# MrGiovanni/R-Super

Hardware: AMD Instinct MI355X
Metric: CT voxels/sec/node (96³ patch, bs=2/GPU) (higher is better)
Workload: dtype bf16; 1 GPU; R-Super 3D UNet(base 32, 26 classes, BasicBlock/IN) full training step (fwd + masked BCE + Dice loss + bwd + clip + AdamW + EMA), 96^3 patches, batch 2/GPU (BASELINE.json configs[1]); global_batch=2, patch=96, parallelism=dp1, sanity_checks_form=device-side flags read one step late (train_ddp.StepGuard)

## Files before the change

include/rsuper_hip.h:

```cpp
#ifndef RSUPER_HIP_H
#define RSUPER_HIP_H
#include <stddef.h>
#include <stdint.h>
#ifdef __cplusplus
extern "C" {
#endif

#define RSUPER_F32 0
#define RSUPER_BF16 1
#define RSUPER_OK 0
#define RSUPER_ERR_ARG 1
#define RSUPER_ERR_LAUNCH 2
#define RSUPER_ERR_UNSUPPORTED 3
#define RSUPER_ERR_NO_DEVICE 4

const char* rsuper_version(void);
int rsuper_device_check(void);


size_t rsuper_conv3_packed_elems(int dtype, int ka, int kb, int n_cols, int bn);

int rsuper_conv3_pack_weights(int dtype, int mode, const float* wa, const float* wb, int ka, int kb, int na, int nb,
                              int bn, void* packed, void* stream);

// ... 56 lines not shown

int rsuper_conv3_wgrad_s2_splits(int dtype, int Ca, int Mtot, int N, int FD, int FH, int FW);
int rsuper_conv3_wgrad_s2(int dtype, const void* xa, int lda, int Ca, const float* mra,
                          const void* ya, int ldya, int Ya, const void* yb, int ldyb, int Yb,
                          float* dwa, float* dwb, float* workspace, int N, int FD, int FH, int FW, int splits, void* stream);

size_t rsuper_pointwise_packed_bytes(int dtype, int K, int N);
int rsuper_pointwise(int dtype, int mode, const float* x, int ldx, const float* w, const float* bias, const float* res, int ldr,
                     float* y, int ldy, long R, int K, int N, void* packed, void* stream);
int rsuper_pointwise_pack_batch(int dtype, const long long* table, int n, long total_items, void* arena, void* stream);
int rsuper_pointwise_wgrad_splits(long R, int N, int K);
int rsuper_pointwise_wgrad(int dtype, const float* dy, int ldy, const float* x, int ldx, long R, int N, int K, float* workspace, int splits,
                           float* dw, float* db, void* stream);

int rsuper_stats_finalize(const float* part, int N, int nblk, int C, double cnt, float eps, int mode, int split, float* out, void* stream);
int rsuper_in_bwd_finalize(int dtype, const void* g, int ldg, const void* x, int ldx, const float* mr, const float* gm,
                           const void* add1, int lda1, const void* add2, int lda2, void* out, int ldo,
                           int N, int vox, int C, void* stream);

int rsuper_maxpool2_fwd(int dtype, const void* x, int ldx, void* y, int ldy, float* part, int blocks,
                        int N, int D, int H, int W, int C, void* stream);
int rsuper_maxpool2_bwd(int dtype, const void* x, int ldx, const void* dy, int lddy, void* dx, int lddx,
                        int N, int D, int H, int W, int C, void* stream);
int rsuper_maxpool2_bwd_add(int dtype, const void* x, int ldx, const void* dy, int lddy, const void* add, int lda, void* dx, int lddx,
                            int N, int D, int H, int W, int C, void* stream);

int rsuper_subsample2_fwd(int dtype, const void* x, int ldx, void* y, int ldy, float* part, int blocks,
                          int N, int D, int H, int W, int C, void* stream);
int rsuper_subsample2_bwd(int dtype, const void* dy, int lddy, void* dx, int lddx, int N, int D, int H, int W, int C, void* stream);

// ... 127 lines not shown
```

r-super_amd/csrc/api.hip:

```cpp
#include <string.h>
#include <math.h>
#include <stdlib.h>
#include "common.hpp"
#include "kernels.hpp"
#include "misc.hpp"
#include "loss.hpp"
#include "morph.hpp"
#include "optim.hpp"
#include "../../include/rsuper_hip.h"

#define ST(s) ((hipStream_t)(s))

static inline bool dt_ok(int dt) { return dt == RS_F32 || dt == RS_BF16; }
static inline bool ch_ok(int C, int ld) { return C >= 0 && (C % 8) == 0 && (ld % 8) == 0 && ld >= C; }
static inline bool bn_ok(int bn) { return bn == 32 || bn == 64 || bn == 96 || bn == 128; }
static inline int ntiles_for(int n_cols, int bn) { const int per = bn / 32; return ((n_cols + bn - 1) / bn) * per; }
static inline int pack_cols(int mode, int na, int nb) { return mode == 1 ? (nb ? (nb & 0xFFFF) : na) : na + nb; }
static inline bool pack_range_ok(int mode, int na, int nb) { return mode != 1 || nb == 0 || ((nb >> 16) % 32 == 0 && (nb & 0xFFFF) > 0 && (nb >> 16) + (nb & 0xFFFF) <= na); }

#include "igemm_plan.hpp"

template <typename F>
static int for_chunks(int n, void* const* p, void* const* g, void* const* m, void* const* v, void* const* e, const size_t* numel, F f) {
    for (int i0 = 0; i0 < n; i0 += RS_MT_MAX) {
// ... 342 lines not shown
}
int rsuper_pointwise_wgrad_splits(long R, int N, int K) { return (R > 0 && R <= 0x7FFFFFFFl && N > 0 && K > 0) ? rs_pw_wgrad_splits((int)R, N, K) : 0; }
int rsuper_pointwise_wgrad(int dtype, const float* dy, int ldy, const float* x, int ldx, long R, int N, int K, float* workspace, int splits,
                           float* dw, float* db, void* stream) {
    if (!dt_ok(dtype) || !dy || !x || !workspace || !dw || R <= 0 || N <= 0 || K <= 0 || splits <= 0) return RS_ERR_ARG;
    if ((N % 4) || (K % 4) || ldy < N || ldx < K) return RS_ERR_ARG;
    if ((unsigned long long)(R + 1) * ldx * 4ull >= (1ull << 32) || (unsigned long long)(R + 1) * ldy * 4ull >= (1ull << 32)) return RS_ERR_UNSUPPORTED;
    return rs_launch_pointwise_wgrad(dtype, dy, ldy, x, ldx, (int)R, N, K, workspace, splits, dw, db, ST(stream));
}

int rsuper_stats_finalize(const float* part, int N, int nblk, int C, double cnt, float eps, int mode, int split, float* out, void* stream) {
    if (!part || !out || N <= 0 || nblk <= 0 || C <= 0 || cnt <= 0 || split < 0 || split >= C || (mode != 0 && mode != 1)) return RS_ERR_ARG;
    return rs_launch_stats_finalize(part, N, nblk, C, cnt, eps, mode, split, out, ST(stream));
}

int rsuper_in_bwd_finalize(int dtype, const void* g, int ldg, const void* x, int ldx, const float* mr, const float* gm,
                           const void* add1, int lda1, const void* add2, int lda2, void* out, int ldo,
                           int N, int vox, int C, void* stream) {
    if (!dt_ok(dtype) || !g || !x || !mr || !gm || !out || !ch_ok(C, ldg) || !ch_ok(C, ldx) || !ch_ok(C, ldo)) return RS_ERR_ARG;
    InBwdParams p = {g, ldg, x, ldx, mr, gm, add1, lda1, add2, lda2, out, ldo, N, vox, C};
    return rs_launch_in_bwd(p, dtype, ST(stream));
}

int rsuper_maxpool2_fwd(int dtype, const void* x, int ldx, void* y, int ldy, float* part, int blocks,
                        int N, int D, int H, int W, int C, void* stream) {
    if (!dt_ok(dtype) || !x || !y || !ch_ok(C, ldx) || !ch_ok(C, ldy) || blocks <= 0 || D < 2 || H < 2 || W < 2) return RS_ERR_ARG;
    PoolParams p = {x, ldx, y, ldy, nullptr, 0, part, N, D, H, W, C};
    return rs_launch_pool(p, dtype, 0, blocks, ST(stream));
}
int rsuper_maxpool2_bwd(int dtype, const void* x, int ldx, const void* dy, int lddy, void* dx, int lddx,
// ... 394 lines not shown
```

r-super_amd/csrc/loss.hip:

```cpp
#include "common.hpp"
#include "misc.hpp"
#include "loss.hpp"

namespace {

__device__ __forceinline__ void sig_bce(float x, float t, float& sg, float& bce) {
    const float e = __expf(-fabsf(x));
    const float r = __frcp_rn(1.f + e);
    sg = x >= 0.f ? r : e * r;
    bce = fmaxf(x, 0.f) - x * t + __logf(1.f + e);
}
__device__ __forceinline__ float sigmoidf(float x) { float s, b; sig_bce(x, 0.f, s, b); return s; }

__global__ __launch_bounds__(256) void plane_partials_fwd_kernel(PlaneParams p) {
    const int plane = blockIdx.y;
    const size_t base = (size_t)plane * p.V;
    const float* x = p.x + (size_t)plane * p.xstride;
    const uint8_t* t = p.tpk ? p.tpk + ((size_t)(plane / p.tC) * p.tP + (size_t)((plane % p.tC) >> 3)) * p.V : (p.t ? p.t + base : nullptr);
    const uint32_t tm8 = p.tpk ? (0x80u >> ((plane % p.tC) & 7)) : 0xFFu;
    const bool kskip = p.kinv && p.kflags && !p.kflags[plane];
    const uint8_t* k = (p.k && !kskip) ? p.k + base : nullptr;
    const int kinv = k ? p.kinv : 0;
    const float* w1 = p.w1 ? p.w1 + base : nullptr;
    const uint8_t* w2 = p.w2 ? p.w2 + base : nullptr;
    float s[6] = {0.f, 0.f, 0.f, 0.f, 0.f, 0.f};
    const bool vec_ok = (p.V & 3) == 0 && (p.xstride & 3) == 0;
    size_t i0 = ((size_t)blockIdx.x * 256 + threadIdx.x) * 4;
    const bool wide_ok = vec_ok && (p.V & 15) == 0 && !w1 &&
                         ((((uintptr_t)p.x | (uintptr_t)p.t | (uintptr_t)p.tpk | (uintptr_t)p.k | (uintptr_t)p.w2) & 15) == 0);
    if (wide_ok) {
        auto term = [&](float xv, uint32_t tb, uint32_t kb, uint32_t w2b) {
            const float tt = (tb & tm8) ? 1.f : 0.f, kk = ((kb != 0u) != (kinv != 0)) ? 1.f : 0.f;
            float sg, b;
            sig_bce(xv, tt, sg, b);
            b *= kk;
            s[0] += b; s[1] += sg * kk; s[2] += sg * tt * kk; s[3] += tt * kk; s[5] += b * (w2b ? 0.f : 1.f);
        };
        for (size_t i = ((size_t)blockIdx.x * 256 + threadIdx.x) * 16; i < (size_t)p.V; i += (size_t)gridDim.x * 256 * 16) {
            float4 q[4];
#pragma unroll
            for (int u = 0; u < 4; ++u) q[u] = *(const float4*)(x + i + 4 * u);
            const uint4 tq = t ? *(const uint4*)(t + i) : make_uint4(0, 0, 0, 0);
            const uint4 kq = k ? *(const uint4*)(k + i) : make_uint4(0x01010101u, 0x01010101u, 0x01010101u, 0x01010101u);
            const uint4 wq = w2 ? *(const uint4*)(w2 + i) : make_uint4(0, 0, 0, 0);
            const uint32_t tw[4] = {tq.x, tq.y, tq.z, tq.w}, kw[4] = {kq.x, kq.y, kq.z, kq.w}, ww[4] = {wq.x, wq.y, wq.z, wq.w};
#pragma unroll
            for (int u = 0; u < 4; ++u) {
                const float xv[4] = {q[u].x, q[u].y, q[u].z, q[u].w};
#pragma unroll
                for (int j = 0; j < 4; ++j) term(xv[j], (tw[u] >> (8 * j)) & 0xFFu, (kw[u] >> (8 * j)) & 0xFFu, (ww[u] >> (8 * j)) & 0xFFu);
            }
        }
        i0 = (size_t)p.V;
    }
    for (size_t i = i0; i < (size_t)p.V; i += (size_t)gridDim.x * 256 * 4) {
        float xv[4]; uint8_t tv[4] = {0, 0, 0, 0}, kv[4] = {1, 1, 1, 1}, w2v[4] = {0, 0, 0, 0}; float w1v[4] = {0.f, 0.f, 0.f, 0.f};
        const bool full = vec_ok && i + 4 <= (size_t)p.V;
        if (full) {
            const float4 q = *(const float4*)(x + i);
            xv[0] = q.x; xv[1] = q.y; xv[2] = q.z; xv[3] = q.w;
            if (t) { const uchar4 u = *(const uchar4*)(t + i); tv[0] = u.x; tv[1] = u.y; tv[2] = u.z; tv[3] = u.w; }
            if (k) { const uchar4 u = *(const uchar4*)(k + i); kv[0] = u.x; kv[1] = u.y; kv[2] = u.z; kv[3] = u.w; }
            if (w2) { const uchar4 u = *(const uchar4*)(w2 + i); w2v[0] = u.x; w2v[1] = u.y; w2v[2] = u.z; w2v[3] = u.w; }
            if (w1) { const float4 u = *(const float4*)(w1 + i); w1v[0] = u.x; w1v[1] = u.y; w1v[2] = u.z; w1v[3] = u.w; }
        }
#pragma unroll
// ... 251 lines not shown
}

int rs_plane_partials_blocks(size_t V) {
    int blocks = (int)((V + 4095) / 4096);
    if (blocks > 64) blocks = 64;
    if (blocks < 1) blocks = 1;
    return blocks;
}
int rs_launch_plane_sums_reduce(const double* pblk, int rows, int nb, float* out, hipStream_t st) {
    hipLaunchKernelGGL(plane_sums_reduce_kernel, dim3((unsigned)((rows * 6 + 255) / 256)), dim3(256), 0, st, pblk, rows, nb, out);
    return rs_check_launch();
}
int rs_launch_plane_partials(const PlaneParams& p, int planes, int bwd, hipStream_t st) {
    const int blocks = rs_plane_partials_blocks(p.V);
    if (!bwd) {
        hipLaunchKernelGGL(plane_partials_fwd_kernel, dim3(blocks, planes), dim3(256), 0, st, p);
    } else {
        int b2 = (int)((p.V + 1023) / 1024);
        if (b2 > 256) b2 = 256;
        hipLaunchKernelGGL(plane_partials_bwd_kernel, dim3(b2, planes), dim3(256), 0, st, p);
    }
    return rs_check_launch();
}

int rs_launch_seg_from_sums(const SegSumsParams& p, hipStream_t st) {
    hipLaunchKernelGGL(seg_from_sums_kernel, dim3(1), dim3(256), 0, st, p);
    return rs_check_launch();
}

int rs_launch_report_from_sums(const ReportSumsParams& p, int R, hipStream_t st) {
    hipLaunchKernelGGL(report_from_sums_kernel, dim3(1), dim3(64), 0, st, p, R);
// ... 19 lines not shown
```

r-super_amd/csrc/misc.hpp:

```cpp
#pragma once
#include <hip/hip_runtime.h>
#include <stddef.h>
#include <stdint.h>

struct InBwdParams {
    const void* g; int ldg;
    const void* x; int ldx;
    const float* mr;
    const float* gm;
    const void* add1; int lda1;
    const void* add2; int lda2;
    void* out; int ldo;
    int N, vox, C;
};

struct PoolParams {
    const void* x; int ldx;
    void* y; int ldy;
    void* dx; int lddx;
    float* part;
    int N, D, H, W, C;
    const void* add; int lda;
};

// ... 31 lines not shown
int rs_battn_chunks(int L, int heads);
int rs_launch_battn(const float* fqv, const float* mqv, float* fout, float* mout, float* lse, const float* dfo, const float* dmo,
                    float* dfqv, float* dmqv, float* part, float* pms, int B, int L, int T, int heads, int dh, float scale, int bwd,
                    hipStream_t st);
int rs_launch_se_forward(const float* x, const float* w1, const float* b1, const float* w2, const float* b2, float* part, float* ms, float* tab,
                         float* hbuf, float* y, int N, long vox, int C, int r, hipStream_t st);
int rs_launch_se_backward(const float* x, const float* dy, const float* ident, const float* w1, const float* w2, const float* ms, const float* tab,
                          const float* hbuf, float* part, float* gm, float* dz1buf, float* tab2, float* dx, float* dw1, float* db1, float* dw2,
                          float* db2, int N, long vox, int C, int r, hipStream_t st);
int rs_launch_cl_planar(const float* src, float* dst, int N, long vox, int C, int K, int dir, hipStream_t st);
int rs_depthwise_rows(long vox);
int rs_launch_depthwise(const float* x, const float* w, float* y, int N, int D, int H, int W, int C, int flip, hipStream_t st);
int rs_launch_depthwise_wgrad(const float* x, const float* dy, float* part, float* dw, int N, int D, int H, int W, int C, hipStream_t st);
int rs_launch_stats_finalize(const float* part, int N, int nblk, int C, double cnt, float eps, int mode, int split, float* out, hipStream_t st);
int rs_elem_blocks(size_t items);
int rs_launch_in_bwd(const InBwdParams& p, int dtype, hipStream_t st);
int rs_launch_pool(const PoolParams& p, int dtype, int bwd, int blocks, hipStream_t st);
int rs_launch_subsample(const PoolParams& p, int dtype, int bwd, int blocks, hipStream_t st);
int rs_launch_upsample(const UpParams& p, int dtype, int bwd, int blocks, hipStream_t st);
int rs_launch_stem(const StemParams& p, int dtype, int wgrad, hipStream_t st);
int rs_launch_head(const HeadParams& p, int dtype, int which, hipStream_t st);
```

r-super_amd/csrc/unet_misc.hip:

```cpp
#include <string.h>
#include "common.hpp"
#include "kernels.hpp"
#include "misc.hpp"

namespace {

__global__ __launch_bounds__(1024) void stats_finalize_kernel(const float* part, int nblk, int C, double cnt, float eps, int mode, int split, float* out) {
    __shared__ double red[32][32][2];
    const int n = blockIdx.y;
    const int cl = threadIdx.x & 31, g = threadIdx.x >> 5;
    const int c = blockIdx.x * 32 + cl;
    double s0 = 0.0, s1 = 0.0;
    if (c < C) {
        const float* base = part + ((size_t)n * nblk * C + c) * 2;
        int b = g;
        for (; b + 96 < nblk; b += 128) {
            const float2 v0 = *(const float2*)(base + (size_t)b * C * 2), v1 = *(const float2*)(base + (size_t)(b + 32) * C * 2);
            const float2 v2 = *(const float2*)(base + (size_t)(b + 64) * C * 2), v3 = *(const float2*)(base + (size_t)(b + 96) * C * 2);
            s0 += ((double)v0.x + (double)v1.x) + ((double)v2.x + (double)v3.x);
            s1 += ((double)v0.y + (double)v1.y) + ((double)v2.y + (double)v3.y);
        }
        for (; b < nblk; b += 32) {
            const float2 v = *(const float2*)(base + (size_t)b * C * 2);
            s0 += (double)v.x; s1 += (double)v.y;
// ... 82 lines not shown
            float a[KP];
            unpack16<T>(a1q, a);
#pragma unroll
            for (int j = 0; j < KP; ++j) o[j] += a[j];
        }
        if (a2p) {
            float a[KP];
            unpack16<T>(a2q, a);
#pragma unroll
            for (int j = 0; j < KP; ++j) o[j] += a[j];
        }
        *(uint4*)(op + (size_t)v * p.ldo + c) = pack16<T>(o);
    }
}

template <typename T>
__global__ void maxpool_fwd_kernel(PoolParams p) {
    constexpr int KP = Elem<T>::KP;
    const int CV = p.C / KP, VL = 256 / CV;
    const int vl = threadIdx.x / CV, s = threadIdx.x % CV;
    const bool active = vl < VL;
    const int n = blockIdx.y;
    const int OD = p.D / 2, OH = p.H / 2, OW = p.W / 2;
    const int ovox = OD * OH * OW;
    const int per_blk = (ovox + gridDim.x - 1) / gridDim.x;
    const int v0 = blockIdx.x * per_blk, v1 = min(ovox, v0 + per_blk);
    float s1[KP], s2[KP];
#pragma unroll
    for (int j = 0; j < KP; ++j) { s1[j] = 0.f; s2[j] = 0.f; }
    if (active)
// ... 5 lines not shown
#pragma unroll
            for (int k = 0; k < 8; ++k) {
                const int d = od * 2 + (k >> 2), h = oh * 2 + ((k >> 1) & 1), w = ow * 2 + (k & 1);
                float x[KP];
                unpack16<T>(*(const uint4*)((const T*)p.x + ((((size_t)n * p.D + d) * p.H + h) * p.W + w) * (size_t)p.ldx + s * KP), x);
#pragma unroll
                for (int j = 0; j < KP; ++j) m[j] = fmaxf(m[j], x[j]);
            }
            *(uint4*)((T*)p.y + ((size_t)n * ovox + v) * p.ldy + s * KP) = pack16<T>(m);
#pragma unroll
            for (int j = 0; j < KP; ++j) { s1[j] += m[j]; s2[j] += m[j] * m[j]; }
        }
    if (p.part) block_channel_sums<KP>(s1, s2, p.C, CV, VL, vl, s, active, p.part + ((size_t)n * gridDim.x + blockIdx.x) * p.C * 2);
}

template <typename T>
__global__ void maxpool_bwd_kernel(PoolParams p) {
    constexpr int KP = Elem<T>::KP;
    const int CV = p.C / KP;
    const int n = blockIdx.y;
    const int OD = p.D / 2, OH = p.H / 2, OW = p.W / 2;
    const size_t total = (size_t)OD * OH * OW * CV;
    for (size_t i = (size_t)blockIdx.x * blockDim.x + threadIdx.x; i < total; i += (size_t)gridDim.x * blockDim.x) {
        const int s = (int)(i % CV); const int v = (int)(i / CV);
        const int ow = v % OW, oh = (v / OW) % OH, od = v / (OW * OH);
        float x[8][KP], m[KP], dy[KP];
#pragma unroll
        for (int j = 0; j < KP; ++j) m[j] = -INFINITY;
#pragma unroll
        for (int k = 0; k < 8; ++k) {
// ... 19 lines not shown
            if (p.add) {
                float a[KP];
                unpack16<T>(*(const uint4*)((const T*)p.add + ((((size_t)n * p.D + d) * p.H + h) * p.W + w) * (size_t)p.lda + s * KP), a);
#pragma unroll
                for (int j = 0; j < KP; ++j) o[j] += a[j];
            }
            *(uint4*)((T*)p.dx + ((((size_t)n * p.D + d) * p.H + h) * p.W + w) * (size_t)p.lddx + s * KP) = pack16<T>(o);
        }
    }
}

template <typename T>
__global__ void subsample_fwd_kernel(PoolParams p) {
    constexpr int KP = Elem<T>::KP;
    const int CV = p.C / KP, VL = 256 / CV;
    const int vl = threadIdx.x / CV, s = threadIdx.x % CV;
    const bool active = vl < VL;
    const int n = blockIdx.y;
    const int OD = (p.D + 1) / 2, OH = (p.H + 1) / 2, OW = (p.W + 1) / 2;
    const int ovox = OD * OH * OW;
    const int per_blk = (ovox + gridDim.x - 1) / gridDim.x;
    const int v0 = blockIdx.x * per_blk, v1 = min(ovox, v0 + per_blk);
    float s1[KP], s2[KP];
#pragma unroll
    for (int j = 0; j < KP; ++j) { s1[j] = 0.f; s2[j] = 0.f; }
    if (active)
        for (int v = v0 + vl; v < v1; v += VL) {
            const int ow = v % OW, oh = (v / OW) % OH, od = v / (OW * OH);
            const uint4 q = *(const uint4*)((const T*)p.x + ((((size_t)n * p.D + 2 * od) * p.H + 2 * oh) * p.W + 2 * ow) * (size_t)p.ldx + s * KP);
            *(uint4*)((T*)p.y + ((size_t)n * ovox + v) * p.ldy + s * KP) = q;
            float m[KP];
            unpack16<T>(q, m);
#pragma unroll
            for (int j = 0; j < KP; ++j) { s1[j] += m[j]; s2[j] += m[j] * m[j]; }
        }
    if (p.part) block_channel_sums<KP>(s1, s2, p.C, CV, VL, vl, s, active, p.part + ((size_t)n * gridDim.x + blockIdx.x) * p.C * 2);
}

template <typename T>
__global__ void subsample_bwd_kernel(PoolParams p) {
    constexpr int KP = Elem<T>::KP;
    const int CV = p.C / KP;
    const int n = blockIdx.y;
    const int OH = (p.H + 1) / 2, OW = (p.W + 1) / 2, OD = (p.D + 1) / 2;
    const size_t total = (size_t)p.D * p.H * p.W * CV;
    for (size_t i = (size_t)blockIdx.x * blockDim.x + threadIdx.x; i < total; i += (size_t)gridDim.x * blockDim.x) {
        const int s = (int)(i % CV); const size_t v = i / CV;
        const int w = (int)(v % p.W), h = (int)((v / p.W) % p.H), d = (int)(v / ((size_t)p.W * p.H));
        uint4 q = make_uint4(0, 0, 0, 0);
        if (!((d | h | w) & 1))
            q = *(const uint4*)((const T*)p.y + (((size_t)n * OD + d / 2) * OH + h / 2) * OW * (size_t)p.ldy + (size_t)(w / 2) * p.ldy + s * KP);
// ... 201 lines not shown
                    unpack16<T>(q[k], x);
#pragma unroll
                    for (int j = 0; j < KP; ++j) acc[j] = fmaf(wt[k], x[j], acc[j]);
                }
            }
#pragma unroll
            for (int j = 0; j < KP; ++j) acc[j] = Elem<T>::rnd(acc[j]);
            *(uint4*)(yout + (size_t)v * p.ldy) = pack16<T>(acc);
#pragma unroll
            for (int j = 0; j < KP; ++j) { s1[j] += acc[j]; s2[j] += acc[j] * acc[j]; }
            ow += VL;
            while (ow >= p.OW) { ow -= p.OW; if (++oh == p.OH) { oh = 0; ++od; } }
        }
    }
    if (p.part) block_channel_sums<KP>(s1, s2, p.C, CV, VL, vl, s, active, p.part + ((size_t)n * gridDim.x + blockIdx.x) * p.C * 2);
}

constexpr int UP_MAXW = 12;
struct UpEnt { int lo, n; float w[UP_MAXW]; };
template <typename T, int NW>
__device__ __forceinline__ void up_bwd_rows(const UpParams& p, const UpEnt* td, const UpEnt* th, const UpEnt* tw, int n, uint32_t i0, uint32_t total,
                                            uint32_t stride) {
    constexpr int KP = Elem<T>::KP;
    const uint32_t CV = (uint32_t)p.C / KP;
    const uint32_t ovox = (uint32_t)(p.OD * p.OH * p.OW);
    const __amdgpu_buffer_rsrc_t rs = __builtin_amdgcn_make_buffer_rsrc((void*)((const T*)p.y + (size_t)n * ovox * p.ldy), 0,
                                                                        ovox * (uint32_t)p.ldy * (uint32_t)sizeof(T), 0x00020000);
    for (uint32_t i = i0; i < total; i += stride) {
        const uint32_t v = i / CV, s = i - v * CV;
        const uint32_t iw = v % (uint32_t)p.IW, t2 = v / (uint32_t)p.IW, ih = t2 % (uint32_t)p.IH, id = t2 / (uint32_t)p.IH;
// ... 628 lines not shown
    if (smem > 64 * 1024) (void)hipFuncSetAttribute((const void*)k, hipFuncAttributeMaxDynamicSharedMemorySize, (int)smem);
}

}

int rs_launch_stats_finalize(const float* part, int N, int nblk, int C, double cnt, float eps, int mode, int split, float* out, hipStream_t st) {
    hipLaunchKernelGGL(stats_finalize_kernel, dim3((C + 31) / 32, N), dim3(1024), 0, st, part, nblk, C, cnt, eps, mode, split, out);
    return rs_check_launch();
}

int rs_elem_blocks(size_t items) {
    size_t b = (items + 255) / 256;
    return (int)(b < 1 ? 1 : (b > 4096 ? 4096 : b));
}

int rs_launch_in_bwd(const InBwdParams& p, int dtype, hipStream_t st) {
    const int KP = dtype == RS_F32 ? 4 : 8;
    if ((size_t)p.vox * (p.C / KP) >= 0xFFFFFFFFull) return RS_ERR_UNSUPPORTED;
    const int blocks = rs_elem_blocks((size_t)p.vox * (p.C / KP));
    if (dtype == RS_F32) hipLaunchKernelGGL(in_bwd_finalize_kernel<float>, dim3(blocks, p.N), dim3(256), 0, st, p);
    else hipLaunchKernelGGL(in_bwd_finalize_kernel<bf16_t>, dim3(blocks, p.N), dim3(256), 0, st, p);
    return rs_check_launch();
}

int rs_launch_pool(const PoolParams& p, int dtype, int bwd, int blocks, hipStream_t st) {
    const int KP = dtype == RS_F32 ? 4 : 8;
    const int CV = p.C / KP;
    if (CV > 256) return RS_ERR_UNSUPPORTED;
    if (!bwd) {
        const size_t smem = (size_t)(256 / CV) * p.C * 2 * sizeof(float);
        if (dtype == RS_F32) hipLaunchKernelGGL(maxpool_fwd_kernel<float>, dim3(blocks, p.N), dim3(256), smem, st, p);
        else hipLaunchKernelGGL(maxpool_fwd_kernel<bf16_t>, dim3(blocks, p.N), dim3(256), smem, st, p);
    } else {
        const int b = rs_elem_blocks((size_t)(p.D / 2) * (p.H / 2) * (p.W / 2) * CV);
        if (dtype == RS_F32) hipLaunchKernelGGL(maxpool_bwd_kernel<float>, dim3(b, p.N), dim3(256), 0, st, p);
        else hipLaunchKernelGGL(maxpool_bwd_kernel<bf16_t>, dim3(b, p.N), dim3(256), 0, st, p);
    }
    return rs_check_launch();
}

int rs_launch_subsample(const PoolParams& p, int dtype, int bwd, int blocks, hipStream_t st) {
    const int KP = dtype == RS_F32 ? 4 : 8;
    const int CV = p.C / KP;
    if (CV > 256) return RS_ERR_UNSUPPORTED;
    if (!bwd) {
        const size_t smem = (size_t)(256 / CV) * p.C * 2 * sizeof(float);
        if (dtype == RS_F32) hipLaunchKernelGGL(subsample_fwd_kernel<float>, dim3(blocks, p.N), dim3(256), smem, st, p);
        else hipLaunchKernelGGL(subsample_fwd_kernel<bf16_t>, dim3(blocks, p.N), dim3(256), smem, st, p);
    } else {
        const int b = rs_elem_blocks((size_t)p.D * p.H * p.W * CV);
        if (dtype == RS_F32) hipLaunchKernelGGL(subsample_bwd_kernel<float>, dim3(b, p.N), dim3(256), 0, st, p);
        else hipLaunchKernelGGL(subsample_bwd_kernel<bf16_t>, dim3(b, p.N), dim3(256), 0, st, p);
    }
    return rs_check_launch();
}

static int launch_upsample_bwd4(const void* g, int ldg, void* dx, int lddx, int N, int ID, int IH, int IW, int OD, int OH, int OW, int C, hipStream_t st) {
    static const bool off = getenv("RSUPER_UPSAMPLE_BWD4") && atoi(getenv("RSUPER_UPSAMPLE_BWD4")) == 0;
    if (off || (C % 8) || N > 65535) return RS_ERR_UNSUPPORTED;
    if ((size_t)OD * OH * OW * (size_t)ldg * 2 >= 0xFFFFFFFFull) return RS_ERR_UNSUPPORTED;
    struct Memo { int k[6]; int ok, nmax; };
    static thread_local Memo memo[8] = {};
    static thread_local int memo_next = 0;
// ... 14 lines not shown
    const int nbx = (IW * (C / 8) + 255) / 256;
    const unsigned blocks = (unsigned)(((ID + 1) / 2) * ((IH + 1) / 2) * nbx);
    if (nmax <= 4) hipLaunchKernelGGL((upsample_bwd4_kernel<4>), dim3(blocks, N), dim3(256), 0, st, p, nbx);
    else hipLaunchKernelGGL((upsample_bwd4_kernel<6>), dim3(blocks, N), dim3(256), 0, st, p, nbx);
    return rs_check_launch();
}

int rs_launch_upsample(const UpParams& p, int dtype, int bwd, int blocks, hipStream_t st) {
    const int KP = dtype == RS_F32 ? 4 : 8;
    const int CV = p.C / KP;
    if (CV > 256) return RS_ERR_UNSUPPORTED;
    if (!bwd) {
        static const bool v1 = getenv("RSUPER_UPSAMPLE_V1") != nullptr;
        const size_t smem = (size_t)(256 / CV) * p.C * 2 * sizeof(float);
        const bool small = (size_t)p.N * p.ID * p.IH * p.IW * p.ldx < 0x7FFFFFFFull;
        if (v1 || !small) {
            if (dtype == RS_F32) hipLaunchKernelGGL(upsample_fwd_kernel<float>, dim3(blocks, p.N), dim3(256), smem, st, p);
            else hipLaunchKernelGGL(upsample_fwd_kernel<bf16_t>, dim3(blocks, p.N), dim3(256), smem, st, p);
        } else {
            if (dtype == RS_F32) hipLaunchKernelGGL(upsample_fwd2_kernel<float>, dim3(blocks, p.N), dim3(256), smem, st, p);
            else hipLaunchKernelGGL(upsample_fwd2_kernel<bf16_t>, dim3(blocks, p.N), dim3(256), smem, st, p);
        }
    } else {
        static const bool v1 = getenv("RSUPER_UPSAMPLE_V1") != nullptr;
        auto ratio = [](int O, int I) { return I > 1 ? (double)(O - 1) / (double)(I - 1) : (double)O; };
        const double rmax = fmax(ratio(p.OD, p.ID), fmax(ratio(p.OH, p.IH), ratio(p.OW, p.IW)));
        if (!v1 && 2.0 * rmax + 2.0 > (double)UP_MAXW + 1e-9) return RS_ERR_UNSUPPORTED;
        const int b = rs_elem_blocks((size_t)p.ID * p.IH * p.IW * CV);
        const size_t tab = (size_t)(p.ID + p.IH + p.IW) * sizeof(UpEnt);
        const bool small = (size_t)p.OD * p.OH * p.OW * p.ldy * (dtype == RS_F32 ? 4 : 2) < 0xFFFFFFFFull && (size_t)p.ID * p.IH * p.IW * CV < 0xFFFFFFFFull && tab <= 48 * 1024;
        if (!v1 && dtype == RS_BF16) {
            const int rc = launch_upsample_bwd4(p.y, p.ldy, p.dx, p.lddx, p.N, p.ID, p.IH, p.IW, p.OD, p.OH, p.OW, p.C, st);
            if (rc != RS_ERR_UNSUPPORTED) return rc;
// ... 94 lines not shown
```

r-super_amd/hip/lib.py:

```python
import ctypes
import os
from ctypes import c_int, c_long, c_longlong, c_size_t, c_float, c_double, c_void_p, c_uint32, c_uint

_HERE = os.path.dirname(os.path.abspath(__file__))
SO_PATH = os.path.join(os.path.dirname(_HERE), 'csrc', 'librsuper_hip.so')

F32, BF16 = 0, 1
_LIB = None

P = c_void_p
_SIGS = {
    'rsuper_version': (ctypes.c_char_p, []),
    'rsuper_device_check': (c_int, []),
    'rsuper_conv3_packed_elems': (c_size_t, [c_int] * 5),
    'rsuper_conv3_pack_weights': (c_int, [c_int, c_int, P, P, c_int, c_int, c_int, c_int, c_int, P, P]),
    'rsuper_conv3_pack_weights_batch': (c_int, [c_int, c_int, P, P, P, P, P, P]),
    'rsuper_conv3_tiles': (c_int, [c_int] * 3),
    'rsuper_conv3_variant': (c_int, [c_int]),
    'rsuper_conv3_wgrad2_min_tiles': (c_int, [c_int]),
    'rsuper_conv3_plan': (c_int, [c_int] * 11 + [P]),
    'rsuper_conv3_box_bn': (c_int, [c_int] * 6),
    'rsuper_conv3_kd_bn': (c_int, [c_int] * 8),
    'rsuper_conv3_set_workspace': (c_int, [P, c_size_t]),
    'rsuper_conv3_workspace_bytes': (c_size_t, []),
# ... 8 lines not shown
    'rsuper_conv3_wgrad': (c_int, [c_int, c_int, P, c_int, c_int, P, P, c_int, c_int, P, P, c_int, c_int, P, c_int, c_int,
                                   P, P, P, c_int, c_int, c_int, c_int, c_int, P]),
    'rsuper_conv3_wgrad_partial': (c_int, [c_int, c_int, P, c_int, c_int, P, P, c_int, c_int, P, P, c_int, c_int, P, c_int, c_int,
                                           P, c_int, c_int, c_int, c_int, c_int, P]),
    'rsuper_conv3_wgrad_reduce': (c_int, [P, c_int, c_int, c_int, c_int, P, P, P]),
    'rsuper_conv3_wgrad_reduce_batch': (c_int, [c_int, P, P, P, P, P, P, P, P]),
    'rsuper_conv3_wgrad_reduce_batch_stats': (c_int, [c_int, P, P, P, P, P, P, P, c_int, P, P, P, P, P, P, P, P, c_float, P]),
    'rsuper_conv3_wgrad_s2_splits': (c_int, [c_int] * 7),
    'rsuper_conv3_wgrad_s2': (c_int, [c_int, P, c_int, c_int, P, P, c_int, c_int, P, c_int, c_int, P, P, P, c_int, c_int, c_int, c_int, c_int, P]),
    'rsuper_pointwise_packed_bytes': (c_size_t, [c_int, c_int, c_int]),
    'rsuper_pointwise': (c_int, [c_int, c_int, P, c_int, P, P, P, c_int, P, c_int, c_long, c_int, c_int, P, P]),
    'rsuper_pointwise_pack_batch': (c_int, [c_int, P, c_int, c_long, P, P]),
    'rsuper_pointwise_wgrad_splits': (c_int, [c_long, c_int, c_int]),
    'rsuper_pointwise_wgrad': (c_int, [c_int, P, c_int, P, c_int, c_long, c_int, c_int, P, c_int, P, P, P]),
    'rsuper_stats_finalize': (c_int, [P, c_int, c_int, c_int, c_double, c_float, c_int, c_int, P, P]),
    'rsuper_in_bwd_finalize': (c_int, [c_int, P, c_int, P, c_int, P, P, P, c_int, P, c_int, P, c_int, c_int, c_int, c_int, P]),
    'rsuper_maxpool2_fwd': (c_int, [c_int, P, c_int, P, c_int, P, c_int, c_int, c_int, c_int, c_int, c_int, P]),
    'rsuper_maxpool2_bwd': (c_int, [c_int, P, c_int, P, c_int, P, c_int, c_int, c_int, c_int, c_int, c_int, P]),
    'rsuper_maxpool2_bwd_add': (c_int, [c_int, P, c_int, P, c_int, P, c_int, P, c_int, c_int, c_int, c_int, c_int, c_int, P]),
    'rsuper_subsample2_fwd': (c_int, [c_int, P, c_int, P, c_int, P, c_int, c_int, c_int, c_int, c_int, c_int, P]),
    'rsuper_subsample2_bwd': (c_int, [c_int, P, c_int, P, c_int, c_int, c_int, c_int, c_int, c_int, P]),
    'rsuper_upsample_fwd': (c_int, [c_int, P, c_int, P, c_int, P, c_int] + [c_int] * 8 + [P]),
    'rsuper_upsample_bwd': (c_int, [c_int, P, c_int, P, c_int] + [c_int] * 8 + [P]),
    'rsuper_stem_fwd': (c_int, [c_int, P, P, P, c_int, P, c_int, c_int, c_int, c_int, c_int, P]),
    'rsuper_stem_wgrad': (c_int, [c_int, P, P, c_int, P, c_int, c_int, c_int, c_int, c_int, P]),
    'rsuper_head_fwd': (c_int, [c_int, P, c_int, P, P, P, c_int, c_int, c_int, c_int, P]),
    'rsuper_head_bwd_data': (c_int, [c_int, P, P, P, c_int, c_int, c_int, c_int, c_int, P]),
    'rsuper_head_bwd_weight': (c_int, [c_int, P, c_int, P, P, P, c_int, c_int, c_int, c_int, P]),
    'rsuper_head_bwd': (c_int, [c_int, P, c_int, P, P, P, c_int, P, P, c_int, c_int, c_int, c_int, P]),
    'rsuper_plane_partials_fwd': (c_int, [P, c_size_t, P, P, P, P, P, c_int, c_int, c_size_t, P]),
# ... 105 lines not shown
```

Measured before the change: 172.0 million voxels/s.

## Add tuned glue kernel variants for pooling, upsample, IN backward and loss partials

Adds a runtime-switchable set of alternative glue kernels, enabled by default and disabled by setting RSUPER_GLUE_KERNELS=0. The set includes a software-pipelined loss partials kernel and an unrolled IN-backward finalize with batched loads. It also adds a maxpool forward with multi-voxel load batching, an upsample forward using shared-memory coordinate tables, and a channel split over gridDim.z for small-grid stat kernels. Maxpool backward uses smaller blocks for small grids. The aim is more memory-level parallelism and better occupancy on small late-stage tensors, at the cost of more code paths and extra partial-stat layout complexity.

```diff
diff --git a/include/rsuper_hip.h b/include/rsuper_hip.h
--- a/include/rsuper_hip.h
+++ b/include/rsuper_hip.h
@@ -94,6 +94,7 @@
                            float* dw, float* db, void* stream);
 
 int rsuper_stats_finalize(const float* part, int N, int nblk, int C, double cnt, float eps, int mode, int split, float* out, void* stream);
+int rsuper_glue_variant(int v);
 int rsuper_in_bwd_finalize(int dtype, const void* g, int ldg, const void* x, int ldx, const float* mr, const float* gm,
                            const void* add1, int lda1, const void* add2, int lda2, void* out, int ldo,
                            int N, int vox, int C, void* stream);
diff --git a/r-super_amd/csrc/api.hip b/r-super_amd/csrc/api.hip
--- a/r-super_amd/csrc/api.hip
+++ b/r-super_amd/csrc/api.hip
@@ -380,6 +380,8 @@
     return rs_launch_stats_finalize(part, N, nblk, C, cnt, eps, mode, split, out, ST(stream));
 }
 
+int rsuper_glue_variant(int v) { return rs_glue_variant(v); }
+
 int rsuper_in_bwd_finalize(int dtype, const void* g, int ldg, const void* x, int ldx, const float* mr, const float* gm,
                            const void* add1, int lda1, const void* add2, int lda2, void* out, int ldo,
                            int N, int vox, int C, void* stream) {
diff --git a/r-super_amd/csrc/loss.hip b/r-super_amd/csrc/loss.hip
--- a/r-super_amd/csrc/loss.hip
+++ b/r-super_amd/csrc/loss.hip
@@ -12,6 +12,7 @@
 }
 __device__ __forceinline__ float sigmoidf(float x) { float s, b; sig_bce(x, 0.f, s, b); return s; }
 
+template <bool PIPE>
 __global__ __launch_bounds__(256) void plane_partials_fwd_kernel(PlaneParams p) {
     const int plane = blockIdx.y;
     const size_t base = (size_t)plane * p.V;
@@ -36,20 +37,39 @@
             b *= kk;
             s[0] += b; s[1] += sg * kk; s[2] += sg * tt * kk; s[3] += tt * kk; s[5] += b * (w2b ? 0.f : 1.f);
         };
-        for (size_t i = ((size_t)blockIdx.x * 256 + threadIdx.x) * 16; i < (size_t)p.V; i += (size_t)gridDim.x * 256 * 16) {
-            float4 q[4];
-#pragma unroll
-            for (int u = 0; u < 4; ++u) q[u] = *(const float4*)(x + i + 4 * u);
-            const uint4 tq = t ? *(const uint4*)(t + i) : make_uint4(0, 0, 0, 0);
-            const uint4 kq = k ? *(const uint4*)(k + i) : make_uint4(0x01010101u, 0x01010101u, 0x01010101u, 0x01010101u);
-            const uint4 wq = w2 ? *(const uint4*)(w2 + i) : make_uint4(0, 0, 0, 0);
-            const uint32_t tw[4] = {tq.x, tq.y, tq.z, tq.w}, kw[4] = {kq.x, kq.y, kq.z, kq.w}, ww[4] = {wq.x, wq.y, wq.z, wq.w};
+        struct Trip { float4 q[4]; uint4 tq, kq, wq; };
+        auto fetch = [&](size_t i) {
+            Trip r;
+#pragma unroll
+            for (int u = 0; u < 4; ++u) r.q[u] = *(const float4*)(x + i + 4 * u);
+            r.tq = t ? *(const uint4*)(t + i) : make_uint4(0, 0, 0, 0);
+            r.kq = k ? *(const uint4*)(k + i) : make_uint4(0x01010101u, 0x01010101u, 0x01010101u, 0x01010101u);
+            r.wq = w2 ? *(const uint4*)(w2 + i) : make_uint4(0, 0, 0, 0);
+            return r;
+        };
+        auto eval = [&](const Trip& r) {
+            const uint32_t tw[4] = {r.tq.x, r.tq.y, r.tq.z, r.tq.w}, kw[4] = {r.kq.x, r.kq.y, r.kq.z, r.kq.w}, ww[4] = {r.wq.x, r.wq.y, r.wq.z, r.wq.w};
 #pragma unroll
             for (int u = 0; u < 4; ++u) {
-                const float xv[4] = {q[u].x, q[u].y, q[u].z, q[u].w};
+                const float xv[4] = {r.q[u].x, r.q[u].y, r.q[u].z, r.q[u].w};
 #pragma unroll
                 for (int j = 0; j < 4; ++j) term(xv[j], (tw[u] >> (8 * j)) & 0xFFu, (kw[u] >> (8 * j)) & 0xFFu, (ww[u] >> (8 * j)) & 0xFFu);
             }
+        };
+        const size_t step = (size_t)gridDim.x * 256 * 16;
+        size_t i = ((size_t)blockIdx.x * 256 + threadIdx.x) * 16;
+        if (PIPE) {
+            if (i < (size_t)p.V) {
+                Trip cur = fetch(i);
+                for (i += step; i < (size_t)p.V; i += step) {
+                    const Trip nxt = fetch(i);
+                    eval(cur);
+                    cur = nxt;
+                }
+                eval(cur);
+            }
+        } else {
+            for (; i < (size_t)p.V; i += step) eval(fetch(i));
         }
         i0 = (size_t)p.V;
     }
@@ -331,7 +351,8 @@
 int rs_launch_plane_partials(const PlaneParams& p, int planes, int bwd, hipStream_t st) {
     const int blocks = rs_plane_partials_blocks(p.V);
     if (!bwd) {
-        hipLaunchKernelGGL(plane_partials_fwd_kernel, dim3(blocks, planes), dim3(256), 0, st, p);
+        if (rs_glue_variant(-1)) hipLaunchKernelGGL(plane_partials_fwd_kernel<true>, dim3(blocks, planes), dim3(256), 0, st, p);
+        else hipLaunchKernelGGL(plane_partials_fwd_kernel<false>, dim3(blocks, planes), dim3(256), 0, st, p);
     } else {
         int b2 = (int)((p.V + 1023) / 1024);
         if (b2 > 256) b2 = 256;
diff --git a/r-super_amd/csrc/misc.hpp b/r-super_amd/csrc/misc.hpp
--- a/r-super_amd/csrc/misc.hpp
+++ b/r-super_amd/csrc/misc.hpp
@@ -69,6 +69,7 @@
 int rs_launch_depthwise_wgrad(const float* x, const float* dy, float* part, float* dw, int N, int D, int H, int W, int C, hipStream_t st);
 int rs_launch_stats_finalize(const float* part, int N, int nblk, int C, double cnt, float eps, int mode, int split, float* out, hipStream_t st);
 int rs_elem_blocks(size_t items);
+int rs_glue_variant(int v);
 int rs_launch_in_bwd(const InBwdParams& p, int dtype, hipStream_t st);
 int rs_launch_pool(const PoolParams& p, int dtype, int bwd, int blocks, hipStream_t st);
 int rs_launch_subsample(const PoolParams& p, int dtype, int bwd, int blocks, hipStream_t st);
diff --git a/r-super_amd/csrc/unet_misc.hip b/r-super_amd/csrc/unet_misc.hip
--- a/r-super_amd/csrc/unet_misc.hip
+++ b/r-super_amd/csrc/unet_misc.hip
@@ -120,6 +120,66 @@
     }
 }
 
+template <typename T, int U>
+__global__ __launch_bounds__(256) void in_bwd_finalize2_kernel(InBwdParams p, int cv_shift) {
+    constexpr int KP = Elem<T>::KP;
+    const uint32_t CV = 1u << cv_shift;
+    const uint32_t total = (uint32_t)p.vox * CV;
+    const uint32_t n = blockIdx.y;
+    const uint32_t i0 = blockIdx.x * (256u * U) + threadIdx.x;
+    if (i0 >= total) return;
+    const T* gp = (const T*)p.g + (size_t)n * p.vox * p.ldg;
+    const T* xp = (const T*)p.x + (size_t)n * p.vox * p.ldx;
+    const T* a1p = p.add1 ? (const T*)p.add1 + (size_t)n * p.vox * p.lda1 : nullptr;
+    const T* a2p = p.add2 ? (const T*)p.add2 + (size_t)n * p.vox * p.lda2 : nullptr;
+    T* op = (T*)p.out + (size_t)n * p.vox * p.ldo;
+    const uint32_t c = (i0 & (CV - 1u)) * KP;
+    uint4 gq[U], xq[U], a1q[U], a2q[U];
+#pragma unroll
+    for (int u = 0; u < U; ++u) {
+        const uint32_t i = i0 + 256u * u;
+        const uint32_t v = (i < total ? i : i0) >> cv_shift;
+        gq[u] = *(const uint4*)(gp + (size_t)v * p.ldg + c);
+        xq[u] = *(const uint4*)(xp + (size_t)v * p.ldx + c);
+        a1q[u] = make_uint4(0, 0, 0, 0); a2q[u] = make_uint4(0, 0, 0, 0);
+        if (a1p) a1q[u] = *(const uint4*)(a1p + (size_t)v * p.lda1 + c);
+        if (a2p) a2q[u] = *(const uint4*)(a2p + (size_t)v * p.lda2 + c);
+    }
+    float mu[KP], rs[KP], m1[KP], m2[KP];
+#pragma unroll
+    for (int j = 0; j < KP; ++j) {
+        const size_t o = ((size_t)n * p.C + c + j) * 2;
+        mu[j] = p.mr[o]; rs[j] = p.mr[o + 1]; m1[j] = p.gm[o]; m2[j] = p.gm[o + 1];
+    }
+#pragma unroll
+    for (int u = 0; u < U; ++u) {
+        const uint32_t i = i0 + 256u * u;
+        if (i >= total) break;
+        const uint32_t v = i >> cv_shift;
+        float g[KP], x[KP], o[KP];
+        unpack16<T>(gq[u], g);
+        unpack16<T>(xq[u], x);
+#pragma unroll
+        for (int j = 0; j < KP; ++j) {
+            const float xn = (x[j] - mu[j]) * rs[j];
+            o[j] = rs[j] * (g[j] - m1[j] - xn * m2[j]);
+        }
+        if (a1p) {
+            float a[KP];
+            unpack16<T>(a1q[u], a);
+#pragma unroll
+            for (int j = 0; j < KP; ++j) o[j] += a[j];
+        }
+        if (a2p) {
+            float a[KP];
+            unpack16<T>(a2q[u], a);
+#pragma unroll
+            for (int j = 0; j < KP; ++j) o[j] += a[j];
+        }
+        *(uint4*)(op + (size_t)v * p.ldo + c) = pack16<T>(o);
+    }
+}
+
 template <typename T>
 __global__ void maxpool_fwd_kernel(PoolParams p) {
     constexpr int KP = Elem<T>::KP;
@@ -155,6 +215,58 @@
     if (p.part) block_channel_sums<KP>(s1, s2, p.C, CV, VL, vl, s, active, p.part + ((size_t)n * gridDim.x + blockIdx.x) * p.C * 2);
 }
 
+template <typename T, int U>
+__global__ __launch_bounds__(256) void maxpool_fwd2_kernel(PoolParams p) {
+    constexpr int KP = Elem<T>::KP;
+    const int CV = p.C / KP, VL = 256 / CV;
+    const int CVb = CV / gridDim.z;
+    const int vl = threadIdx.x / CVb, s = blockIdx.z * CVb + threadIdx.x % CVb;
+    const bool active = vl < VL;
+    const int n = blockIdx.y;
+    const int OD = p.D / 2, OH = p.H / 2, OW = p.W / 2;
+    const int ovox = OD * OH * OW;
+    const int per_blk = (ovox + gridDim.x - 1) / gridDim.x;
+    const int v0 = blockIdx.x * per_blk, v1 = min(ovox, v0 + per_blk);
+    float s1[KP], s2[KP];
+#pragma unroll
+    for (int j = 0; j < KP; ++j) { s1[j] = 0.f; s2[j] = 0.f; }
+    if (active)
+        for (int v = v0 + vl; v < v1; v += U * VL) {
+            uint4 q[U][8];
+#pragma unroll
+            for (int u = 0; u < U; ++u) {
+                const int vv = v + u * VL < v1 ? v + u * VL : v;
+                const int ow = vv % OW, oh = (vv / OW) % OH, od = vv / (OW * OH);
+#pragma unroll
+                for (int k = 0; k < 8; ++k) {
+                    const int d = od * 2 + (k >> 2), h = oh * 2 + ((k >> 1) & 1), w = ow * 2 + (k & 1);
+                    q[u][k] = *(const uint4*)((const T*)p.x + ((((size_t)n * p.D + d) * p.H + h) * p.W + w) * (size_t)p.ldx + s * KP);
+                }
+            }
+#pragma unroll
+            for (int u = 0; u < U; ++u) {
+                if (v + u * VL >= v1) break;
+                float m[KP];
+#pragma unroll
+                for (int j = 0; j < KP; ++j) m[j] = -INFINITY;
+#pragma unroll
+                for (int k = 0; k < 8; ++k) {
+                    float x[KP];
+                    unpack16<T>(q[u][k], x);
+#pragma unroll
+                    for (int j = 0; j < KP; ++j) m[j] = fmaxf(m[j], x[j]);
+                }
+                *(uint4*)((T*)p.y + ((size_t)n * ovox + v + u * VL) * p.ldy + s * KP) = pack16<T>(m);
+#pragma unroll
+                for (int j = 0; j < KP; ++j) { s1[j] += m[j]; s2[j] = fmaf(m[j], m[j], s2[j]); }
+            }
+        }
+    const int Cb = CVb * KP;
+    if (p.part)
+        block_channel_sums<KP>(s1, s2, Cb, CVb, VL, vl, threadIdx.x % CVb, active,
+                               p.part + (((size_t)n * gridDim.x + blockIdx.x) * p.C + (size_t)blockIdx.z * Cb) * 2);
+}
+
 template <typename T>
 __global__ void maxpool_bwd_kernel(PoolParams p) {
     constexpr int KP = Elem<T>::KP;
@@ -204,7 +316,8 @@
 __global__ void subsample_fwd_kernel(PoolParams p) {
     constexpr int KP = Elem<T>::KP;
     const int CV = p.C / KP, VL = 256 / CV;
-    const int vl = threadIdx.x / CV, s = threadIdx.x % CV;
+    const int CVb = CV / gridDim.z;
+    const int vl = threadIdx.x / CVb, s = blockIdx.z * CVb + threadIdx.x % CVb;
     const bool active = vl < VL;
     const int n = blockIdx.y;
     const int OD = (p.D + 1) / 2, OH = (p.H + 1) / 2, OW = (p.W + 1) / 2;
@@ -224,7 +337,10 @@
 #pragma unroll
             for (int j = 0; j < KP; ++j) { s1[j] += m[j]; s2[j] += m[j] * m[j]; }
         }
-    if (p.part) block_channel_sums<KP>(s1, s2, p.C, CV, VL, vl, s, active, p.part + ((size_t)n * gridDim.x + blockIdx.x) * p.C * 2);
+    const int Cb = CVb * KP;
+    if (p.part)
+        block_channel_sums<KP>(s1, s2, Cb, CVb, VL, vl, threadIdx.x % CVb, active,
+                               p.part + (((size_t)n * gridDim.x + blockIdx.x) * p.C + (size_t)blockIdx.z * Cb) * 2);
 }
 
 template <typename T>
@@ -456,6 +572,100 @@
         }
     }
     if (p.part) block_channel_sums<KP>(s1, s2, p.C, CV, VL, vl, s, active, p.part + ((size_t)n * gridDim.x + blockIdx.x) * p.C * 2);
+}
+
+struct UpTab { uint32_t o0, o1; float l0, l1; };
+template <typename T>
+__global__ __launch_bounds__(256) void upsample_fwd3_kernel(UpParams p) {
+    extern __shared__ __attribute__((aligned(16))) char smem[];
+    constexpr int KP = Elem<T>::KP;
+    const int CV = p.C / KP, VL = 256 / CV;
+    const int CVb = CV / gridDim.z;
+    const int Cb = CVb * KP;
+    const int vl = threadIdx.x / CVb, s = blockIdx.z * CVb + threadIdx.x % CVb;
+    const bool active = vl < VL;
+    const int n = blockIdx.y;
+    const int ovox = p.OD * p.OH * p.OW;
+    const int per_blk = (ovox + gridDim.x - 1) / gridDim.x;
+    const int v0 = blockIdx.x * per_blk, v1 = min(ovox, v0 + per_blk);
+    const float sd = p.OD > 1 ? (float)(p.ID - 1) / (float)(p.OD - 1) : 0.f;
+    const float sh = p.OH > 1 ? (float)(p.IH - 1) / (float)(p.OH - 1) : 0.f;
+    const float sw = p.OW > 1 ? (float)(p.IW - 1) / (float)(p.OW - 1) : 0.f;
+    UpTab* tab = (UpTab*)(smem + (size_t)VL * Cb * 2 * sizeof(float));
+    for (int t = threadIdx.x; t < p.OD + p.OH + p.OW; t += blockDim.x) {
+        const int axis = t < p.OD ? 0 : (t < p.OD + p.OH ? 1 : 2);
+        const int o = axis == 0 ? t : (axis == 1 ? t - p.OD : t - p.OD - p.OH);
+        const float sc = axis == 0 ? sd : (axis == 1 ? sh : sw);
+        const int I = axis == 0 ? p.ID : (axis == 1 ? p.IH : p.IW);
+        const uint32_t stride = (uint32_t)sizeof(T) * (uint32_t)p.ldx * (axis == 0 ? (uint32_t)(p.IH * p.IW) : (axis == 1 ? (uint32_t)p.IW : 1u));
+        int i0, i1; float l;
+        lin_coord(o, sc, I, i0, i1, l);
+        UpTab e;
+        e.o0 = (uint32_t)i0 * stride; e.o1 = (uint32_t)i1 * stride; e.l0 = 1.f - l; e.l1 = l;
+        tab[t] = e;
+    }
+    __syncthreads();
+    const UpTab* td = tab; const UpTab* th = tab + p.OD; const UpTab* tw = tab + p.OD + p.OH;
+    float s1[KP], s2[KP];
+#pragma unroll
+    for (int j = 0; j < KP; ++j) { s1[j] = 0.f; s2[j] = 0.f; }
+    const char* xin = (const char*)((const T*)p.x + (size_t)n * p.ID * p.IH * p.IW * p.ldx + s * KP);
+    if (active && v0 + vl < v1) {
+        int v = v0 + vl;
+        int ow = v % p.OW, oh = (v / p.OW) % p.OH, od = v / (p.OW * p.OH);
+        T* yp = (T*)p.y + ((size_t)n * ovox + v) * p.ldy + s * KP;
+        const size_t ystep = (size_t)VL * p.ldy;
+        for (; v < v1; v += VL, yp += ystep) {
+            const UpTab ed = td[od], eh = th[oh], ew = tw[ow];
+            const uint32_t rows[4] = {ed.o0 + eh.o0, ed.o0 + eh.o1, ed.o1 + eh.o0, ed.o1 + eh.o1};
+            const float wdh[4] = {ed.l0 * eh.l0, ed.l0 * eh.l1, ed.l1 * eh.l0, ed.l1 * eh.l1};
+            uint4 q[8];
+            float wt[8];
+#pragma unroll
+            for (int k = 0; k < 8; ++k) {
+                q[k] = *(const uint4*)(xin + (rows[k >> 1] + ((k & 1) ? ew.o1 : ew.o0)));
+                wt[k] = wdh[k >> 1] * ((k & 1) ? ew.l1 : ew.l0);
+            }
+            float acc[KP];
+            if (sizeof(T) == 2) {
+                f32x2_t a2[4];
+#pragma unroll
+                for (int j = 0; j < 4; ++j) a2[j] = f32x2_t{0.f, 0.f};
+#pragma unroll
+                for (int k = 0; k < 8; ++k) {
+                    const uint32_t wq[4] = {q[k].x, q[k].y, q[k].z, q[k].w};
+                    const f32x2_t w2 = {wt[k], wt[k]};
+#pragma unroll
+                    for (int j = 0; j < 4; ++j) {
+                        const f32x2_t x2 = {__uint_as_float(wq[j] << 16), __uint_as_float(wq[j] & 0xffff0000u)};
+                        a2[j] = __builtin_elementwise_fma(w2, x2, a2[j]);
+                    }
+                }
+#pragma unroll
+                for (int j = 0; j < 4; ++j) { acc[2 * j] = a2[j][0]; acc[2 * j + 1] = a2[j][1]; }
+            } else {
+#pragma unroll
+                for (int j = 0; j < KP; ++j) acc[j] = 0.f;
+#pragma unroll
+                for (int k = 0; k < 8; ++k) {
+                    float x[KP];
+                    unpack16<T>(q[k], x);
+#pragma unroll
+                    for (int j = 0; j < KP; ++j) acc[j] = fmaf(wt[k], x[j], acc[j]);
+                }
+            }
+#pragma unroll
+            for (int j = 0; j < KP; ++j) acc[j] = Elem<T>::rnd(acc[j]);
+            *(uint4*)yp = pack16<T>(acc);
+#pragma unroll
+            for (int j = 0; j < KP; ++j) { s1[j] += acc[j]; s2[j] = fmaf(acc[j], acc[j], s2[j]); }
+            ow += VL;
+            while (ow >= p.OW) { ow -= p.OW; if (++oh == p.OH) { oh = 0; ++od; } }
+        }
+    }
+    if (p.part)
+        block_channel_sums<KP>(s1, s2, Cb, CVb, VL, vl, threadIdx.x % CVb, active,
+                               p.part + (((size_t)n * gridDim.x + blockIdx.x) * p.C + (size_t)blockIdx.z * Cb) * 2);
 }
 
 constexpr int UP_MAXW = 12;
@@ -1114,10 +1324,39 @@
     return (int)(b < 1 ? 1 : (b > 4096 ? 4096 : b));
 }
 
+int rs_glue_variant(int v) {
+    static int g = !(getenv("RSUPER_GLUE_KERNELS") && atoi(getenv("RSUPER_GLUE_KERNELS")) == 0);
+    if (v == 0 || v == 1) g = v;
+    return g;
+}
+
+static int stat_csplit(int rows, int N, int CV) {
+    if (!rs_glue_variant(-1)) return 1;
+    const int VL = 256 / CV;
+    int z = 1;
+    while ((size_t)rows * N * z < 1024 && CV % (2 * z) == 0 && CV / (2 * z) >= 8 && (CV / (2 * z)) * VL >= 64) z *= 2;
+    return z;
+}
+
 int rs_launch_in_bwd(const InBwdParams& p, int dtype, hipStream_t st) {
     const int KP = dtype == RS_F32 ? 4 : 8;
     if ((size_t)p.vox * (p.C / KP) >= 0xFFFFFFFFull) return RS_ERR_UNSUPPORTED;
     const int blocks = rs_elem_blocks((size_t)p.vox * (p.C / KP));
+    const uint32_t CV = (uint32_t)(p.C / KP);
+    const size_t nb1 = ((size_t)p.vox * CV + 255) / 256;
+    if (rs_glue_variant(-1) && CV > 0 && (CV & (CV - 1)) == 0 && CV <= 256 && nb1 >= 256 && nb1 <= 8192) {
+        const int sh = __builtin_ctz(CV);
+        if (nb1 >= 1024) {
+            const dim3 grid((unsigned)((nb1 + 3) / 4), p.N);
+            if (dtype == RS_F32) hipLaunchKernelGGL((in_bwd_finalize2_kernel<float, 4>), grid, dim3(256), 0, st, p, sh);
+            else hipLaunchKernelGGL((in_bwd_finalize2_kernel<bf16_t, 4>), grid, dim3(256), 0, st, p, sh);
+        } else {
+            const dim3 grid((unsigned)((nb1 + 1) / 2), p.N);
+            if (dtype == RS_F32) hipLaunchKernelGGL((in_bwd_finalize2_kernel<float, 2>), grid, dim3(256), 0, st, p, sh);
+            else hipLaunchKernelGGL((in_bwd_finalize2_kernel<bf16_t, 2>), grid, dim3(256), 0, st, p, sh);
+        }
+        return rs_check_launch();
+    }
     if (dtype == RS_F32) hipLaunchKernelGGL(in_bwd_finalize_kernel<float>, dim3(blocks, p.N), dim3(256), 0, st, p);
     else hipLaunchKernelGGL(in_bwd_finalize_kernel<bf16_t>, dim3(blocks, p.N), dim3(256), 0, st, p);
     return rs_check_launch();
@@ -1129,12 +1368,21 @@
     if (CV > 256) return RS_ERR_UNSUPPORTED;
     if (!bwd) {
         const size_t smem = (size_t)(256 / CV) * p.C * 2 * sizeof(float);
-        if (dtype == RS_F32) hipLaunchKernelGGL(maxpool_fwd_kernel<float>, dim3(blocks, p.N), dim3(256), smem, st, p);
-        else hipLaunchKernelGGL(maxpool_fwd_kernel<bf16_t>, dim3(blocks, p.N), dim3(256), smem, st, p);
+        if (rs_glue_variant(-1) && (size_t)blocks * p.N < 1024) {
+            const int z = stat_csplit(blocks, p.N, CV);
+            const dim3 grid(blocks, p.N, z), blk(z == 1 ? 256 : (CV / z) * (256 / CV));
+            if (dtype == RS_F32) hipLaunchKernelGGL((maxpool_fwd2_kernel<float, 4>), grid, blk, smem / z, st, p);
+            else hipLaunchKernelGGL((maxpool_fwd2_kernel<bf16_t, 4>), grid, blk, smem / z, st, p);
+        } else {
+            if (dtype == RS_F32) hipLaunchKernelGGL(maxpool_fwd_kernel<float>, dim3(blocks, p.N), dim3(256), smem, st, p);
+            else hipLaunchKernelGGL(maxpool_fwd_kernel<bf16_t>, dim3(blocks, p.N), dim3(256), smem, st, p);
+        }
     } else {
-        const int b = rs_elem_blocks((size_t)(p.D / 2) * (p.H / 2) * (p.W / 2) * CV);
-        if (dtype == RS_F32) hipLaunchKernelGGL(maxpool_bwd_kernel<float>, dim3(b, p.N), dim3(256), 0, st, p);
-        else hipLaunchKernelGGL(maxpool_bwd_kernel<bf16_t>, dim3(b, p.N), dim3(256), 0, st, p);
+        const size_t items = (size_t)(p.D / 2) * (p.H / 2) * (p.W / 2) * CV;
+        int b = rs_elem_blocks(items), threads = 256;
+        if (rs_glue_variant(-1) && (size_t)b * p.N < 512) { threads = 64; b = (int)((items + 63) / 64); }
+        if (dtype == RS_F32) hipLaunchKernelGGL(maxpool_bwd_kernel<float>, dim3(b, p.N), dim3(threads), 0, st, p);
+        else hipLaunchKernelGGL(maxpool_bwd_kernel<bf16_t>, dim3(b, p.N), dim3(threads), 0, st, p);
     }
     return rs_check_launch();
 }
@@ -1145,8 +1393,10 @@
     if (CV > 256) return RS_ERR_UNSUPPORTED;
     if (!bwd) {
         const size_t smem = (size_t)(256 / CV) * p.C * 2 * sizeof(float);
-        if (dtype == RS_F32) hipLaunchKernelGGL(subsample_fwd_kernel<float>, dim3(blocks, p.N), dim3(256), smem, st, p);
-        else hipLaunchKernelGGL(subsample_fwd_kernel<bf16_t>, dim3(blocks, p.N), dim3(256), smem, st, p);
+        const int z = stat_csplit(blocks, p.N, CV);
+        const dim3 grid(blocks, p.N, z), blk(z == 1 ? 256 : (CV / z) * (256 / CV));
+        if (dtype == RS_F32) hipLaunchKernelGGL(subsample_fwd_kernel<float>, grid, blk, smem / z, st, p);
+        else hipLaunchKernelGGL(subsample_fwd_kernel<bf16_t>, grid, blk, smem / z, st, p);
     } else {
         const int b = rs_elem_blocks((size_t)p.D * p.H * p.W * CV);
         if (dtype == RS_F32) hipLaunchKernelGGL(subsample_bwd_kernel<float>, dim3(b, p.N), dim3(256), 0, st, p);
@@ -1191,9 +1441,16 @@
         static const bool v1 = getenv("RSUPER_UPSAMPLE_V1") != nullptr;
         const size_t smem = (size_t)(256 / CV) * p.C * 2 * sizeof(float);
         const bool small = (size_t)p.N * p.ID * p.IH * p.IW * p.ldx < 0x7FFFFFFFull;
+        const size_t tab3 = (size_t)(p.OD + p.OH + p.OW) * sizeof(UpTab);
+        const bool fwd3 = rs_glue_variant(-1) && small && (size_t)p.ID * p.IH * p.IW * p.ldx * (dtype == RS_F32 ? 4 : 2) < 0xFFFFFFFFull && smem + tab3 <= 64 * 1024;
         if (v1 || !small) {
             if (dtype == RS_F32) hipLaunchKernelGGL(upsample_fwd_kernel<float>, dim3(blocks, p.N), dim3(256), smem, st, p);
             else hipLaunchKernelGGL(upsample_fwd_kernel<bf16_t>, dim3(blocks, p.N), dim3(256), smem, st, p);
+        } else if (fwd3) {
+            const int z = stat_csplit(blocks, p.N, CV);
+            const dim3 grid(blocks, p.N, z), blk(z == 1 ? 256 : (CV / z) * (256 / CV));
+            if (dtype == RS_F32) hipLaunchKernelGGL(upsample_fwd3_kernel<float>, grid, blk, smem / z + tab3, st, p);
+            else hipLaunchKernelGGL(upsample_fwd3_kernel<bf16_t>, grid, blk, smem / z + tab3, st, p);
         } else {
             if (dtype == RS_F32) hipLaunchKernelGGL(upsample_fwd2_kernel<float>, dim3(blocks, p.N), dim3(256), smem, st, p);
             else hipLaunchKernelGGL(upsample_fwd2_kernel<bf16_t>, dim3(blocks, p.N), dim3(256), smem, st, p);
diff --git a/r-super_amd/hip/lib.py b/r-super_amd/hip/lib.py
--- a/r-super_amd/hip/lib.py
+++ b/r-super_amd/hip/lib.py
@@ -46,6 +46,7 @@
     'rsuper_pointwise_wgrad_splits': (c_int, [c_long, c_int, c_int]),
     'rsuper_pointwise_wgrad': (c_int, [c_int, P, c_int, P, c_int, c_long, c_int, c_int, P, c_int, P, P, P]),
     'rsuper_stats_finalize': (c_int, [P, c_int, c_int, c_int, c_double, c_float, c_int, c_int, P, P]),
+    'rsuper_glue_variant': (c_int, [c_int]),
     'rsuper_in_bwd_finalize': (c_int, [c_int, P, c_int, P, c_int, P, P, P, c_int, P, c_int, P, c_int, c_int, c_int, c_int, P]),
     'rsuper_maxpool2_fwd': (c_int, [c_int, P, c_int, P, c_int, P, c_int, c_int, c_int, c_int, c_int, c_int, P]),
     'rsuper_maxpool2_bwd': (c_int, [c_int, P, c_int, P, c_int, P, c_int, c_int, c_int, c_int, c_int, c_int, P]),
```

Result: faster. 174.2 million voxels/s, median of 6 (+1.3%).
